# pasqualedem/LabelAnything

Hardware: AMD Instinct MI355X
Metric: episodes/sec (query+support fwd) ViT-B 1024px 1-shot (higher is better)
Workload: dtype f16; 1 GPU; BASELINE cfg2: SAM ViT-B 1024px encoder + LabelAnything decoder, 1-way 1-shot episodes (2 images each), random-init weights, full-resolution logits; parallelism=episode-sharded x1, no collective, launch=hipGraph replay

## Files before the change

labelanything_amd/csrc/attn_enc.hip:

```cpp
#include <cstdlib>
#include "la_common.h"
#ifndef LA_ATTN_ABL
#ifndef LA_ATTN_DMA_RUN
#define LA_ATTN_DMA_RUN 1
#endif
#define LA_ATTN_ABL 0
#endif
#ifndef LA_WIN_ROT
#define LA_WIN_ROT 1
#endif
#ifndef LA_WIN_HALF
#define LA_WIN_HALF 1
#endif
#ifndef LA_ATTN_X
#define LA_ATTN_X 0
#endif
#include "../../include/la_hip.h"
#include "attn_plan.h"

namespace la {

constexpr int HD = 64;
constexpr float NEG_BIG = -1.0e30f;
constexpr float RESCALE_THR = 8.0f;

template <typename T, int NH>
__global__ __launch_bounds__(256) void relpos_kernel(const T* __restrict__ qkv, int B, int heads, int G, int E,
                                                     const T* __restrict__ tabh, const T* __restrict__ tabw,
                                                     float* __restrict__ relh, float* __restrict__ relw) {
  const int w = blockIdx.x * 4 + (threadIdx.x >> 6);
  if (w >= B * heads * G) return;
  const int lane = threadIdx.x & 63, fr = lane & 31, fh = lane >> 5;
  const int y = w % G, bh = w / G, h = bh % heads, b = bh / heads;
  const int T_ = G * G;
  const int ntx = (G + 31) >> 5;
  const uint4 zero = make_uint4(0, 0, 0, 0);

  constexpr int HDT = 64 * NH, KS = 4 * NH;
  uint4 af[2][KS];
#pragma unroll
  for (int ti = 0; ti < 2; ++ti) {
    const int x = ti * 32 + fr;
    const bool ok = (ti < ntx) && (x < G);
    const T* p = qkv + ((size_t)b * T_ + (size_t)y * G + (ok ? x : 0)) * (3 * E) + h * HDT + fh * 8;
#pragma unroll
    for (int ks = 0; ks < KS; ++ks) af[ti][ks] = ok ? *reinterpret_cast<const uint4*>(p + ks * 16) : zero;
  }
  const size_t obase = ((size_t)bh * T_ + (size_t)y * G) * G;

  for (int tj = 0; tj < ntx; ++tj) {
    const int j = tj * 32 + fr;
    const bool okj = j < G;
    const T* p = tabh + (size_t)(okj ? (y - j + G - 1) : 0) * HDT + fh * 8;
    uint4 wf[KS];
#pragma unroll
    for (int ks = 0; ks < KS; ++ks) wf[ks] = okj ? *reinterpret_cast<const uint4*>(p + ks * 16) : zero;
#pragma unroll
    for (int ti = 0; ti < 2; ++ti) {
      if (ti >= ntx) continue;
      f32x16 acc;
#pragma unroll
      for (int r = 0; r < 16; ++r) acc[r] = 0.f;
#pragma unroll
      for (int ks = 0; ks < KS; ++ks) acc = Half16<T>::mfma32(af[ti][ks], wf[ks], acc);
#pragma unroll
      for (int r = 0; r < 16; ++r) {
        const int x = ti * 32 + (r & 3) + 8 * (r >> 2) + 4 * fh;
        if (x < G && okj) relh[obase + (size_t)x * G + j] = acc[r];
      }
    }
  }
  const int nrel = 2 * G - 1;
  const int ntr = (nrel + 31) >> 5;
  for (int tj = 0; tj < ntr; ++tj) {
    const int rp = tj * 32 + fr;
    const bool okr = rp < nrel;
    const T* p = tabw + (size_t)(okr ? rp : 0) * HDT + fh * 8;
    uint4 wf[KS];
#pragma unroll
    for (int ks = 0; ks < KS; ++ks) wf[ks] = okr ? *reinterpret_cast<const uint4*>(p + ks * 16) : zero;
#pragma unroll
    for (int ti = 0; ti < 2; ++ti) {
      if (ti >= ntx) continue;
      f32x16 acc;
#pragma unroll
      for (int r = 0; r < 16; ++r) acc[r] = 0.f;
#pragma unroll
      for (int ks = 0; ks < KS; ++ks) acc = Half16<T>::mfma32(af[ti][ks], wf[ks], acc);
#pragma unroll
      for (int r = 0; r < 16; ++r) {
        const int x = ti * 32 + (r & 3) + 8 * (r >> 2) + 4 * fh;
        const int kw = x + G - 1 - rp;
        if (x < G && okr && kw >= 0 && kw < G) relw[obase + (size_t)x * G + kw] = acc[r];
      }
    }
  }
}


__device__ __forceinline__ float xhalf_max(float v) {
  const auto r = __builtin_amdgcn_permlane32_swap(__float_as_uint(v), __float_as_uint(v), false, false);
  return fmaxf(__uint_as_float(r[0]), __uint_as_float(r[1]));
}
__device__ __forceinline__ float xhalf_sum(float v) {
  const auto r = __builtin_amdgcn_permlane32_swap(__float_as_uint(v), __float_as_uint(v), false, false);
  return __uint_as_float(r[0]) + __uint_as_float(r[1]);
}

#ifdef LA_DEBUG
__device__ unsigned long long g_win_stamps[4 * 16];
#define WIN_STAMP(i)                                                                                  \
  do {                                                                                                \
    if (MODE == ATTN_TABLES_WIN16 && blockIdx.x == gridDim.x / 2) {                                   \
      unsigned long long t_;                                                                          \
      asm volatile("s_memtime %0\n\ts_waitcnt lgkmcnt(0)" : "=s"(t_)::"memory");                     \
      if ((threadIdx.x & 63) == 0) g_win_stamps[(threadIdx.x >> 6) * 16 + (i)] = t_;                   \
    }                                                                                                 \
  } while (0)
#else
#define WIN_STAMP(i) do {} while (0)
#endif

struct AttnArgs {
  const void* qkv;
  const void* vt;
  void* out;
  const float* relh;
  const float* relw;
  const void* tabh;
  const void* tabw;
  int B, heads, T, Tpad, G, E;
  float scale;
  float* lse;
  float* cspart;
  int csH, csW;
  int imgH, imgW;
  const void* padrow;
  int nwx, nwin;
  unsigned mg_heads, mg_nwin, mg_nwx, mg_G;
};

__device__ __forceinline__ int udiv_magic(int n, int d, unsigned magic) { return d == 1 ? n : (int)__umulhi((unsigned)n, magic); }
static inline unsigned magic_of(int d) { return d <= 1 ? 0u : (unsigned)((0x100000000ull + (unsigned)d - 1) / (unsigned)d); }
static inline void set_win_magic(AttnArgs& a) {
  a.nwx = a.imgH > 0 ? (a.imgW + a.G - 1) / a.G : 1;
  a.nwin = a.imgH > 0 ? a.nwx * ((a.imgH + a.G - 1) / a.G) : 1;
  a.mg_heads = magic_of(a.heads);
  a.mg_nwin = magic_of(a.nwin);
  a.mg_nwx = magic_of(a.nwx);
  a.mg_G = magic_of(a.G);
}

template <typename T, int MODE, int NH, bool VROW = false>
__global__ __launch_bounds__(256, (((MODE == ATTN_TABLES_ROW64 || MODE == ATTN_TABLES_WIN16) && NH == 1) ? 3 : 2)) void attn_fwd_kernel(AttnArgs a) {
  constexpr bool WIN16 = MODE == ATTN_TABLES_WIN16;
  constexpr bool ROW64 = MODE == ATTN_TERMS_ROW64 || MODE == ATTN_TABLES_ROW64;
  constexpr int HDT = 64 * NH, KS = 4 * NH, SUB = 64 * 64 * 2, KVS = KV_STAGE * NH;
  extern __shared__ __attribute__((aligned(16))) char smem[];
  WIN_STAMP(0);
  const int tid = threadIdx.x, lane = tid & 63, wave = tid >> 6;
  const int fr = lane & 31, fh = lane >> 5;
  const int BH = a.B * a.heads;
  int bh, qblk;
  {
    const int nq = (a.T + 127) / 128;
    if (WIN16) {
      const bool two = nq == 2;
      if ((BH & 7) == 0) {
        const int idx = blockIdx.x >> 3;
        qblk = two ? (idx & 1) : 0;
        bh = ((two ? idx >> 1 : idx) << 3) + (blockIdx.x & 7);
      } else {
        qblk = (int)blockIdx.x >= BH;
        bh = blockIdx.x - (qblk ? BH : 0);
      }
    } else if ((BH & 7) == 0) {
      const int idx = blockIdx.x >> 3;
      qblk = idx % nq;
      bh = (idx / nq) * 8 + (blockIdx.x & 7);
    } else {
      bh = blockIdx.x % BH;
      qblk = blockIdx.x / BH;
    }
  }
  const int b = WIN16 ? udiv_magic(bh, a.heads, a.mg_heads) : bh / a.heads;
  const int h = bh - b * a.heads;
  const int T_ = a.T, E3 = 3 * a.E;
  const T* qkv = reinterpret_cast<const T*>(a.qkv);
  const T* vt = reinterpret_cast<const T*>(a.vt);
  const int q0 = qblk * 128 + ((WIN16 && LA_WIN_ROT) ? ((wave + bh) & 3) : wave) * 32;
  const int q = q0 + fr;
  const int qc = min(q, T_ - 1);
  const float inv_scale = 1.0f / a.scale;
  const float c2 = a.scale * 1.44269504088896340736f;
  const bool img_order = WIN16 && VROW && a.imgH > 0;
  int wimg = 0, wy0 = 0, wx0 = 0;
  if (img_order) {
    wimg = udiv_magic(b, a.nwin, a.mg_nwin);
    const int w_ = b - wimg * a.nwin;
    const int wy = udiv_magic(w_, a.nwx, a.mg_nwx);
    wy0 = wy * a.G;
    wx0 = (w_ - wy * a.nwx) * a.G;
  }
  const int qy5 = WIN16 ? udiv_magic(qc, a.G, a.mg_G) : 0, qx5 = qc - qy5 * a.G;
  auto img_row = [&](int ty, int tx) -> long {
    const int y = wy0 + ty, x = wx0 + tx;
    return (y < a.imgH && x < a.imgW) ? ((long)wimg * a.imgH + y) * a.imgW + x : -1;
  };
  long qrow = (long)b * T_ + qc;
  if (img_order) qrow = img_row(qy5, qx5);
  const T* padrow = reinterpret_cast<const T*>(a.padrow);
  if (img_order && a.lse == nullptr && wy0 + udiv_magic(qblk * 128, a.G, a.mg_G) >= a.imgH) {
    if (a.cspart != nullptr && tid < HDT) a.cspart[((size_t)b * ((T_ + 127) / 128) + qblk) * a.E + h * HDT + tid] = 0.f;
    return;
  }

  uint4 qf[KS];
  {
    const T* p = (qrow >= 0 ? qkv + (size_t)qrow * E3 : padrow) + h * HDT + fh * 8;
#pragma unroll
    for (int ks = 0; ks < KS; ++ks) qf[ks] = *reinterpret_cast<const uint4*>(p + ks * 16);
  }

  const T* ksrc[2];
  const T* vsrc[2];
  int krow[2], koff[2], voff[2];
#pragma unroll
  for (int i = 0; i < 2; ++i) {
    const int row = (i * 4 + wave) * 8 + (lane >> 3);
    const int chunk = (lane & 7) ^ ((row >> 1) & 7);
    krow[i] = row;
    koff[i] = a.E + h * HDT + chunk * 8;
    voff[i] = 2 * a.E + h * HDT + ((lane & 7) ^ (4 * ((row >> 1) & 1))) * 8;
    ksrc[i] = qkv + (size_t)b * T_ * E3 + koff[i];
    vsrc[i] = VROW ? qkv + (size_t)b * T_ * E3 + voff[i] : vt + ((size_t)bh * HDT + row) * a.Tpad + chunk * 8;
  }
  const unsigned lds0 = lds_addr_of(smem);
  const T* img_base = qkv + (size_t)b * T_ * E3;
  unsigned krun[2], vrun[2];
#pragma unroll
  for (int i = 0; i < 2; ++i) {
    krun[i] = (unsigned)(((size_t)krow[i] * E3 + koff[i]) * sizeof(T));
    vrun[i] = (unsigned)(((size_t)krow[i] * E3 + voff[i]) * sizeof(T));
  }
  const unsigned tile_step = (unsigned)((size_t)64 * E3 * sizeof(T));
  auto dma = [&](int j, int stage) {
    const unsigned sk = lds0 + stage * KVS;
    const unsigned sv = sk + NH * SUB;
#pragma unroll
    for (int i = 0; i < 2; ++i) {
      int key = 0;
      const T* kp = nullptr;
      const T* vp = nullptr;
      if (!WIN16 && !LA_ATTN_DMA_RUN) {
        key = min(j * 64 + krow[i], T_ - 1);
        kp = ksrc[i] + (size_t)key * E3;
        if (VROW) vp = vsrc[i] + (size_t)key * E3;
      } else if (!WIN16) {
        unsigned ko = krun[i], vo = vrun[i];
        if (j * 64 + 64 > T_) {
          const unsigned back = (unsigned)max(j * 64 + krow[i] - (T_ - 1), 0) * (unsigned)(E3 * sizeof(T));
          ko -= back;
          vo -= back;
        }
        krun[i] += tile_step;
        vrun[i] += tile_step;
#pragma unroll
        for (int hh = 0; hh < NH; ++hh) {
          dma16s(img_base, ko + hh * 128, sk + hh * SUB + (i * 4 + wave) * 1024);
          if (VROW) dma16s(img_base, vo + hh * 128, sv + hh * SUB + (i * 4 + wave) * 1024);
          else dma16(vsrc[i] + (size_t)hh * 64 * a.Tpad + j * 64, sv + hh * SUB + (i * 4 + wave) * 1024);
        }
        continue;
      } else if (WIN16) {
        const int slot = j * 64 + krow[i];
        const int ty = min(slot >> 4, a.G - 1), tx = min(slot & 15, a.G - 1);
        key = ty * a.G + tx;
        if (img_order) {
          const long r = img_row(ty, tx);
          const T* rp = r >= 0 ? qkv + (size_t)r * E3 : padrow;
          kp = rp + koff[i];
          vp = rp + voff[i];
        }
      }
      if (WIN16 && !img_order) {
        kp = ksrc[i] + (size_t)key * E3;
        if (VROW) vp = vsrc[i] + (size_t)key * E3;
      }
#pragma unroll
      for (int hh = 0; hh < NH; ++hh) {
        dma16(kp + hh * 64, sk + hh * SUB + (i * 4 + wave) * 1024);
        if (VROW) dma16(vp + hh * 64, sv + hh * SUB + (i * 4 + wave) * 1024);
        else dma16(vsrc[i] + (size_t)hh * 64 * a.Tpad + j * 64, sv + hh * SUB + (i * 4 + wave) * 1024);
      }
    }
  };

  const int ntiles = WIN16 ?((16 * a.G + 63) >> 6) : ((T_ + 63) >> 6);
  const bool half_last = WIN16 && LA_WIN_HALF && ((16 * a.G) & 63) != 0 && ((16 * a.G) & 63) <= 32;
  dma(0, 0);
  WIN_STAMP(1);

  float* bias_lds = reinterpret_cast<float*>(smem + 2 * KVS);
  f32x16 rw[2];
  float bw8[8];
  float* my_bh = nullptr;
  float* my_bw = nullptr;
  const int* keyinfo = nullptr;
  if (MODE == ATTN_TERMS_ROW64) {
    my_bh = bias_lds + wave * 32 * 65;
    for (int i = 0; i < 32; ++i) {
      const int qi = min(q0 + i, T_ - 1);
      my_bh[i * 65 + lane] = a.relh[((size_t)bh * T_ + qi) * 64 + lane] * inv_scale;
    }
    const float* p = a.relw + ((size_t)bh * T_ + qc) * 64;
#pragma unroll
    for (int t = 0; t < 2; ++t)
#pragma unroll
      for (int g4 = 0; g4 < 4; ++g4) {
        const float4 v = *reinterpret_cast<const float4*>(p + t * 32 + 8 * g4 + 4 * fh);
        rw[t][g4 * 4 + 0] = v.x * inv_scale;
        rw[t][g4 * 4 + 1] = v.y * inv_scale;
        rw[t][g4 * 4 + 2] = v.z * inv_scale;
        rw[t][g4 * 4 + 3] = v.w * inv_scale;
      }
  } else if (WIN16) {
    const int G = a.G, nrel = 2 * G - 1;
    my_bh = bias_lds + wave * 32 * 33;
    const T* th = reinterpret_cast<const T*>(a.tabh) + (size_t)min(fr, nrel - 1) * HDT + fh * 8;
    const T* tw = reinterpret_cast<const T*>(a.tabw) + (size_t)min(fr, nrel - 1) * HDT + fh * 8;
    f32x16 uh, uw;
#pragma unroll
    for (int r = 0; r < 16; ++r) uh[r] = uw[r] = 0.f;
#pragma unroll
    for (int ks = 0; ks < KS; ++ks) {
      uh = Half16<T>::mfma32(*reinterpret_cast<const uint4*>(th + ks * 16), qf[ks], uh);
      uw = Half16<T>::mfma32(*reinterpret_cast<const uint4*>(tw + ks * 16), qf[ks], uw);
    }
#pragma unroll
    for (int r = 0; r < 16; ++r) my_bh[fr * 33 + (r & 3) + 8 * (r >> 2) + 4 * fh] = uw[r] * inv_scale;
    __builtin_amdgcn_wave_barrier();
    const int qx = qx5;
#pragma unroll
    for (int i = 0; i < 8; ++i) {
      const int kw = 8 * (i >> 2) + 4 * fh + (i & 3);
      bw8[i] = (kw < G) ? my_bh[fr * 33 + qx + G - 1 - kw] : NEG_BIG;
    }
    __builtin_amdgcn_wave_barrier();
#pragma unroll
    for (int r = 0; r < 16; ++r) my_bh[fr * 33 + (r & 3) + 8 * (r >> 2) + 4 * fh] = uh[r] * inv_scale;
    __builtin_amdgcn_wave_barrier();
  } else if (MODE == ATTN_TABLES_ROW64) {
    my_bh = bias_lds + wave * 32 * 33;
    const int x0 = q0 & 63;
    const T* tabw = reinterpret_cast<const T*>(a.tabw);
#pragma unroll
    for (int t = 0; t < 2; ++t)
#pragma unroll
      for (int r = 0; r < 16; ++r) rw[t][r] = 0.f;
#pragma unroll 1
    for (int tt = 0; tt < 3; ++tt) {
      const T* tp = tabw + (size_t)min(x0 + tt * 32 + fr, 126) * HDT + fh * 8;
      f32x16 u;
#pragma unroll
      for (int r = 0; r < 16; ++r) u[r] = 0.f;
#pragma unroll
      for (int ks = 0; ks < KS; ++ks) u = Half16<T>::mfma32(*reinterpret_cast<const uint4*>(tp + ks * 16), qf[ks], u);
      __builtin_amdgcn_wave_barrier();
#pragma unroll
      for (int r = 0; r < 16; ++r) my_bh[fr * 33 + (r & 3) + 8 * (r >> 2) + 4 * fh] = u[r] * inv_scale;
      __builtin_amdgcn_wave_barrier();
#pragma unroll
      for (int t = 0; t < 2; ++t)
#pragma unroll
        for (int r = 0; r < 16; ++r) {
          const int kw = t * 32 + (r & 3) + 8 * (r >> 2) + 4 * fh;
          const int i = fr + 63 - kw - tt * 32;
          if (i >= 0 && i < 32) rw[t][r] = my_bh[fr * 33 + i];
        }
    }
    __builtin_amdgcn_wave_barrier();
  } else if (MODE == ATTN_TERMS) {
    const int G = a.G, GS = G + 1;
    my_bh = bias_lds + wave * 2 * 32 * GS;
    my_bw = my_bh + 32 * GS;
    for (int idx = lane; idx < 32 * G; idx += 64) {
      const int i = idx / G, k = idx % G;
      const size_t src = ((size_t)bh * T_ + min(q0 + i, T_ - 1)) * G + k;
      my_bh[i * GS + k] = a.relh[src] * inv_scale;
      my_bw[i * GS + k] = a.relw[src] * inv_scale;
    }
    int* ki = reinterpret_cast<int*>(bias_lds + 4 * 2 * 32 * GS);
    for (int k = tid; k < a.Tpad; k += 256) ki[k] = ((k / G) << 16) | (k % G);
    keyinfo = ki;
  } else if (MODE == ATTN_TABLES_WIN) {
    const int G = a.G, nrel = 2 * G - 1;
    my_bh = bias_lds + wave * 2 * 32 * 33;
    my_bw = my_bh + 32 * 33;
    const T* th = reinterpret_cast<const T*>(a.tabh) + (size_t)min(fr, nrel - 1) * HDT + fh * 8;
    const T* tw = reinterpret_cast<const T*>(a.tabw) + (size_t)min(fr, nrel - 1) * HDT + fh * 8;
    f32x16 uh, uw;
#pragma unroll
    for (int r = 0; r < 16; ++r) uh[r] = uw[r] = 0.f;
#pragma unroll
    for (int ks = 0; ks < KS; ++ks) {
      uh = Half16<T>::mfma32(*reinterpret_cast<const uint4*>(th + ks * 16), qf[ks], uh);
      uw = Half16<T>::mfma32(*reinterpret_cast<const uint4*>(tw + ks * 16), qf[ks], uw);
    }
#pragma unroll
    for (int r = 0; r < 16; ++r) {
      const int row = (r & 3) + 8 * (r >> 2) + 4 * fh;
      my_bh[fr * 33 + row] = uh[r] * inv_scale;
      my_bw[fr * 33 + row] = uw[r] * inv_scale;
    }
    int* ki = reinterpret_cast<int*>(bias_lds + 4 * 2 * 32 * 33);
    for (int k = tid; k < a.Tpad; k += 256) {
      const int kk = min(k, T_ - 1);
      ki[k] = ((G - 1 - kk / G) << 16) | (G - 1 - kk % G);
    }
    keyinfo = ki;
  }

  f32x16 oacc[2 * NH];
#pragma unroll
  for (int d = 0; d < 2 * NH; ++d)
#pragma unroll
    for (int r = 0; r < 16; ++r) oacc[d][r] = 0.f;
  float m_run = NEG_BIG, l_run = 0.f;
  unsigned vtr[2] = {0u, 0u};
  if (VROW) {
    const int j = (lane & 15) >> 2, c = lane & 3, jb = (j >> 1) & 1, gd = (lane >> 4) & 1;
#pragma unroll
    for (int dd = 0; dd < 2; ++dd) vtr[dd] = (unsigned)((8 * fh + j) * 128 + ((4 * (dd ^ jb) + 2 * gd + (c >> 1)) << 4) + (c & 1) * 8);
  }

  WIN_STAMP(2);
  dma_wait<0>();
  auto fill_relh_half = [&](int hf) {
    const int y = q0 >> 6;
    const T* tp = reinterpret_cast<const T*>(a.tabh) + (size_t)min(y + (1 - hf) * 32 + fr, 126) * HDT + fh * 8;
    f32x16 u;
#pragma unroll
    for (int r = 0; r < 16; ++r) u[r] = 0.f;
#pragma unroll
    for (int ks = 0; ks < KS; ++ks) u = Half16<T>::mfma32(*reinterpret_cast<const uint4*>(tp + ks * 16), qf[ks], u);
    __builtin_amdgcn_wave_barrier();
#pragma unroll
    for (int r = 0; r < 16; ++r) my_bh[fr * 33 + 31 - ((r & 3) + 8 * (r >> 2) + 4 * fh)] = u[r] * inv_scale;
    __builtin_amdgcn_wave_barrier();
  };
  if (MODE == ATTN_TABLES_ROW64) fill_relh_half(0);
  __syncthreads();
  WIN_STAMP(3);
  const bool idle_wave = q0 >= T_;
  for (int j = 0; j < ntiles; ++j) {
#if !(LA_ATTN_ABL & 8)
    if (j + 1 < ntiles) dma(j + 1, (j + 1) & 1);
#endif
    if (idle_wave) {
      dma_wait<0>();
      __syncthreads();
      continue;
    }
    const char* sk = smem + (j & 1) * KVS;
    const char* sv = sk + NH * SUB;
    if (MODE == ATTN_TABLES_ROW64 && j == 32) fill_relh_half(1);

    f32x16 s[2];
    float rh = 0.f;
    const bool half = WIN16 && half_last && j == ntiles - 1;
    if (MODE == ATTN_TERMS_ROW64) rh = my_bh[fr * 65 + j];
    if (MODE == ATTN_TABLES_ROW64) rh = my_bh[fr * 33 + (j & 31)];
#pragma unroll
    for (int t = 0; t < 2; ++t) {
      if (WIN16 && t == 1 && half) continue;
      const uint4 kf0 = *reinterpret_cast<const uint4*>(sk + swz_off(t * 32 + fr, fh));
      if (ROW64) {
        s[t] = Half16<T>::mfma32(kf0, qf[0], rw[t]);
      } else if (WIN16) {
        f32x16 z;
        const int qy = qy5;
#pragma unroll
        for (int hh = 0; hh < 2; ++hh) {
          const int kh = 4 * j + 2 * t + hh;
          const float bh = (kh < a.G) ? my_bh[fr * 33 + qy + a.G - 1 - kh] : NEG_BIG;
#pragma unroll
          for (int i = 0; i < 8; ++i) z[hh * 8 + i] = bh + bw8[i];
        }
        s[t] = Half16<T>::mfma32(kf0, qf[0], z);
      } else {
        f32x16 z;
#pragma unroll
        for (int r = 0; r < 16; ++r) z[r] = 0.f;
        s[t] = Half16<T>::mfma32(kf0, qf[0], z);
      }
    }
#if !(LA_ATTN_ABL & 2)
#pragma unroll
    for (int ks = 1; ks < KS; ++ks) {
#pragma unroll
      for (int t = 0; t < 2; ++t) {
        if (WIN16 && t == 1 && half) continue;
        const uint4 kf = *reinterpret_cast<const uint4*>(sk + (ks >> 2) * SUB + swz_off(t * 32 + fr, (ks & 3) * 2 + fh));
        s[t] = Half16<T>::mfma32(kf, qf[ks], s[t]);
      }
    }
#endif
    if (MODE == ATTN_TERMS) {
      const int GS = a.G + 1;
#pragma unroll
      for (int t = 0; t < 2; ++t)
#pragma unroll
        for (int r = 0; r < 16; ++r) {
          const int key = j * 64 + t * 32 + (r & 3) + 8 * (r >> 2) + 4 * fh;
          const int info = keyinfo[key];
          s[t][r] += my_bh[fr * GS + (info >> 16)] + my_bw[fr * GS + (info & 0xffff)];
        }
    }
    if (MODE == ATTN_TABLES_WIN) {
      const int qy = qc / a.G, qx = qc % a.G;
      const float* bh_q = my_bh + fr * 33 + qy;
      const float* bw_q = my_bw + fr * 33 + qx;
#pragma unroll
      for (int t = 0; t < 2; ++t)
#pragma unroll
        for (int r = 0; r < 16; ++r) {
          const int key = j * 64 + t * 32 + (r & 3) + 8 * (r >> 2) + 4 * fh;
          const int info = keyinfo[key];
          s[t][r] += bh_q[info >> 16] + bw_q[info & 0xffff];
        }
    }
    if (!WIN16 && j * 64 + 64 > T_) {
#pragma unroll
      for (int t = 0; t < 2; ++t)
#pragma unroll
        for (int r = 0; r < 16; ++r) {
          const int key = j * 64 + t * 32 + (r & 3) + 8 * (r >> 2) + 4 * fh;
          if (key >= T_) s[t][r] = NEG_BIG;
        }
    }

#if LA_ATTN_X & 2
    if (j == 0) {
#endif
    float mx = s[0][0];
#pragma unroll
    for (int t = 0; t < 2; ++t) {
      if (WIN16 && t == 1 && half) continue;
#pragma unroll
      for (int r = 0; r < 16; ++r) mx = fmaxf(mx, s[t][r]);
    }
    mx = xhalf_max(mx) + rh;
    if (!__all((mx - m_run) * c2 <= RESCALE_THR)) {
      const float m_new = fmaxf(m_run, mx);
      const float alpha = __builtin_amdgcn_exp2f((m_run - m_new) * c2);
      l_run *= alpha;
#pragma unroll
      for (int d = 0; d < 2 * NH; ++d)
#pragma unroll
        for (int r = 0; r < 16; ++r) oacc[d][r] *= alpha;
      m_run = m_new;
    }
#if LA_ATTN_X & 2
    }
#endif
    const float mc = (rh - m_run) * c2;
    float psum = 0.f;
#pragma unroll
    for (int t = 0; t < 2; ++t) {
      if (WIN16 && t == 1 && half) continue;
#pragma unroll
      for (int r = 0; r < 16; ++r) {
#if LA_ATTN_ABL & 1
        const float p = fmaf(s[t][r], c2, mc);
#else
#if LA_ATTN_X & 4
        const float p = __builtin_amdgcn_exp2f(s[t][r]);
#else
        const float p = __builtin_amdgcn_exp2f(fmaf(s[t][r], c2, mc));
#endif
#endif
        s[t][r] = p;
#if !(LA_ATTN_X & 8)
        psum += p;
#endif
      }
    }
    l_run += psum;

    uint4 pf[4];
#pragma unroll
    for (int ks = 0; ks < 4; ++ks) {
      if (WIN16 && ks >= 2 && half) continue;
      const int t = ks >> 1, g0 = (ks & 1) * 8;
      const uint32_t x0 = pack2<T>(s[t][g0 + 0], s[t][g0 + 1]);
      const uint32_t x1 = pack2<T>(s[t][g0 + 2], s[t][g0 + 3]);
      const uint32_t y0 = pack2<T>(s[t][g0 + 4], s[t][g0 + 5]);
      const uint32_t y1 = pack2<T>(s[t][g0 + 6], s[t][g0 + 7]);
      const auto r0 = __builtin_amdgcn_permlane32_swap(x0, y0, false, false);
      const auto r1 = __builtin_amdgcn_permlane32_swap(x1, y1, false, false);
      pf[ks] = make_uint4(r0[0], r1[0], r0[1], r1[1]);
    }

#if LA_ATTN_ABL & 4
    asm volatile("" ::"v"(pf[0].x), "v"(pf[0].y), "v"(pf[0].z), "v"(pf[0].w), "v"(pf[1].x), "v"(pf[1].y), "v"(pf[1].z), "v"(pf[1].w));
    asm volatile("" ::"v"(pf[2].x), "v"(pf[2].y), "v"(pf[2].z), "v"(pf[2].w), "v"(pf[3].x), "v"(pf[3].y), "v"(pf[3].z), "v"(pf[3].w));
#else
#pragma unroll
    for (int ks = 0; ks < 4; ++ks) {
      if (WIN16 && ks >= 2 && half) continue;
#pragma unroll
      for (int d = 0; d < 2 * NH; ++d) {
        uint4 vf;
        if (VROW) {
          typedef short s16x4 __attribute__((ext_vector_type(4)));
          typedef __attribute__((address_space(3))) s16x4* lds_s16x4;
          const unsigned va = lds_addr_of(sv) + (d >> 1) * SUB + vtr[d & 1] + ks * 2048;
          const s16x4 lo = __builtin_amdgcn_ds_read_tr16_b64_v4i16((lds_s16x4)(uintptr_t)va);
          const s16x4 hi = __builtin_amdgcn_ds_read_tr16_b64_v4i16((lds_s16x4)(uintptr_t)(va + 512));
          const uint2 l2 = __builtin_bit_cast(uint2, lo), h2 = __builtin_bit_cast(uint2, hi);
          vf = make_uint4(l2.x, l2.y, h2.x, h2.y);
        } else {
          vf = *reinterpret_cast<const uint4*>(sv + (d >> 1) * SUB + swz_off((d & 1) * 32 + fr, ks * 2 + fh));
        }
        oacc[d] = Half16<T>::mfma32(vf, pf[ks], oacc[d]);
      }
    }
#endif

#if !(LA_ATTN_ABL & 8)
    if (j < 4) WIN_STAMP(8 + j);
    dma_wait<0>();
    __syncthreads();
#endif
    if (j < 4) WIN_STAMP(4 + j);
  }

  const float l_tot = xhalf_sum(l_run);
  const float inv_l = 1.0f / l_tot;
  if (a.lse != nullptr && q < T_ && fh == 0) a.lse[(size_t)bh * a.Tpad + q] = m_run * c2 + __builtin_amdgcn_logf(l_tot);
  if (q < T_ && qrow >= 0) {
    T* op = reinterpret_cast<T*>(a.out) + (size_t)qrow * a.E + h * HDT;
#pragma unroll
    for (int d = 0; d < 2 * NH; ++d)
#pragma unroll
      for (int g4 = 0; g4 < 4; ++g4) {
        uint2 v;
        v.x = pack2<T>(oacc[d][g4 * 4 + 0] * inv_l, oacc[d][g4 * 4 + 1] * inv_l);
        v.y = pack2<T>(oacc[d][g4 * 4 + 2] * inv_l, oacc[d][g4 * 4 + 3] * inv_l);
        *reinterpret_cast<uint2*>(op + d * 32 + 8 * g4 + 4 * fh) = v;
      }
  }
  WIN_STAMP(12);
  if (a.cspart != nullptr) {
    bool valid = q < T_ && qrow >= 0;
    if (WIN16 && a.csH > 0 && !img_order) {
      const int nwx = (a.csW + a.G - 1) / a.G, nwy = (a.csH + a.G - 1) / a.G;
      const int w = b % (nwx * nwy);
      valid = valid && (w / nwx) * a.G + qy5 < a.csH && (w % nwx) * a.G + qx5 < a.csW;
    }
    char* tile = smem + wave * (NH * 4096);
#pragma unroll
    for (int d = 0; d < 2 * NH; ++d)
#pragma unroll
      for (int g4 = 0; g4 < 4; ++g4) {
        uint2 v;
        v.x = pack2<T>(oacc[d][g4 * 4 + 0] * inv_l, oacc[d][g4 * 4 + 1] * inv_l);
        v.y = pack2<T>(oacc[d][g4 * 4 + 2] * inv_l, oacc[d][g4 * 4 + 3] * inv_l);
        if (!valid) v = make_uint2(0u, 0u);
        const int c16 = 4 * (d & 1) + g4;
        *reinterpret_cast<uint2*>(tile + (d >> 1) * 4096 + fr * 128 + ((c16 ^ (4 * ((fr >> 1) & 1))) << 4) + 8 * fh) = v;
      }
    asm volatile("s_waitcnt lgkmcnt(0)" ::: "memory");
    __builtin_amdgcn_wave_barrier();
    unsigned ctr[2];
    {
      const int j = (lane & 15) >> 2, c = lane & 3, jb = (j >> 1) & 1, gd = (lane >> 4) & 1;
#pragma unroll
      for (int dd = 0; dd < 2; ++dd) ctr[dd] = (unsigned)((8 * fh + j) * 128 + ((4 * (dd ^ jb) + 2 * gd + (c >> 1)) << 4) + (c & 1) * 8);
    }
    const uint32_t one2 = pack2<T>(1.0f, 1.0f);
    const uint4 ones = make_uint4(one2, one2, one2, one2);
    float* red = reinterpret_cast<float*>(smem + 4 * NH * 4096);
#pragma unroll
    for (int d = 0; d < 2 * NH; ++d) {
      f32x16 cs;
#pragma unroll
      for (int r = 0; r < 16; ++r) cs[r] = 0.f;
#pragma unroll
      for (int ks = 0; ks < 2; ++ks) {
        typedef short s16x4 __attribute__((ext_vector_type(4)));
        typedef __attribute__((address_space(3))) s16x4* lds_s16x4;
        const unsigned va = lds_addr_of(tile) + (d >> 1) * 4096 + ctr[d & 1] + ks * 2048;
        const s16x4 lo = __builtin_amdgcn_ds_read_tr16_b64_v4i16((lds_s16x4)(uintptr_t)va);
        const s16x4 hi = __builtin_amdgcn_ds_read_tr16_b64_v4i16((lds_s16x4)(uintptr_t)(va + 512));
        const uint2 l2 = __builtin_bit_cast(uint2, lo), h2 = __builtin_bit_cast(uint2, hi);
        cs = Half16<T>::mfma32(make_uint4(l2.x, l2.y, h2.x, h2.y), ones, cs);
      }
      if (fr == 0) {
#pragma unroll
        for (int r = 0; r < 16; ++r) red[wave * HDT + d * 32 + (r & 3) + 8 * (r >> 2) + 4 * fh] = cs[r];
      }
    }
    __syncthreads();
    if (tid < HDT) {
      float t = 0.f;
#pragma unroll
      for (int w = 0; w < 4; ++w) t += red[w * HDT + tid];
      const int nq = (T_ + 127) / 128;
      a.cspart[((size_t)b * nq + qblk) * a.E + h * HDT + tid] = t;
    }
  }
}


template <typename T>
__global__ __launch_bounds__(256, 3) void attn_window_kernel(AttnArgs a, int qtiles) {
  extern __shared__ __attribute__((aligned(16))) char smem[];
  const int tid = threadIdx.x, lane = tid & 63, wave = tid >> 6;
  const int fr = lane & 31, fh = lane >> 5;
  const int G = a.G, T_ = a.T, E3 = 3 * a.E;
  int* keyinfo = reinterpret_cast<int*>(smem);
  for (int k = tid; k < a.Tpad; k += 256) {
    const int kk = min(k, T_ - 1);
    keyinfo[k] = ((G - 1 - kk / G) << 16) | (G - 1 - kk % G);
  }
  __syncthreads();
  const int job = blockIdx.x * 4 + wave;
  const int njobs = a.B * a.heads * qtiles;
  if (job >= njobs) return;
  const int qt = job % qtiles, bh = job / qtiles;
  const int h = bh % a.heads, b = bh / a.heads;
  const T* qkv = reinterpret_cast<const T*>(a.qkv);
  const T* vt = reinterpret_cast<const T*>(a.vt);
  const int q0 = qt * 32, q = q0 + fr, qc = min(q, T_ - 1);
  const float inv_scale = 1.0f / a.scale;
  const float c2 = a.scale * 1.44269504088896340736f;

  uint4 qf[4];
  {
    const T* p = qkv + ((size_t)b * T_ + qc) * E3 + h * HD + fh * 8;
#pragma unroll
    for (int ks = 0; ks < 4; ++ks) qf[ks] = *reinterpret_cast<const uint4*>(p + ks * 16);
  }
  float* my_bh = reinterpret_cast<float*>(smem + a.Tpad * sizeof(int)) + wave * 2 * 32 * 33;
  float* my_bw = my_bh + 32 * 33;
  {
    const int nrel = 2 * G - 1;
    const T* th = reinterpret_cast<const T*>(a.tabh) + (size_t)min(fr, nrel - 1) * HD + fh * 8;
    const T* tw = reinterpret_cast<const T*>(a.tabw) + (size_t)min(fr, nrel - 1) * HD + fh * 8;
    f32x16 uh, uw;
#pragma unroll
    for (int r = 0; r < 16; ++r) uh[r] = uw[r] = 0.f;
#pragma unroll
    for (int ks = 0; ks < 4; ++ks) {
      uh = Half16<T>::mfma32(*reinterpret_cast<const uint4*>(th + ks * 16), qf[ks], uh);
      uw = Half16<T>::mfma32(*reinterpret_cast<const uint4*>(tw + ks * 16), qf[ks], uw);
    }
#pragma unroll
    for (int r = 0; r < 16; ++r) {
      const int row = (r & 3) + 8 * (r >> 2) + 4 * fh;
      my_bh[fr * 33 + row] = uh[r] * inv_scale;
      my_bw[fr * 33 + row] = uw[r] * inv_scale;
    }
    __builtin_amdgcn_wave_barrier();
  }
  const float* bh_q = my_bh + fr * 33 + qc / G;
  const float* bw_q = my_bw + fr * 33 + qc % G;

  const T* kbase = qkv + (size_t)b * T_ * E3 + a.E + h * HD + fh * 8;
  const T* vbase = vt + ((size_t)bh * HD + fr) * a.Tpad + fh * 8;
  f32x16 oacc[2];
#pragma unroll
  for (int d = 0; d < 2; ++d)
#pragma unroll
    for (int r = 0; r < 16; ++r) oacc[d][r] = 0.f;
  float m_run = NEG_BIG, l_run = 0.f;
  const int ntiles = (T_ + 63) >> 6;
  for (int j = 0; j < ntiles; ++j) {
    f32x16 s[2];
#pragma unroll
    for (int t = 0; t < 2; ++t) {
      const T* kp = kbase + (size_t)min(j * 64 + t * 32 + fr, T_ - 1) * E3;
      uint4 kf[4];
#pragma unroll
      for (int ks = 0; ks < 4; ++ks) kf[ks] = *reinterpret_cast<const uint4*>(kp + ks * 16);
#pragma unroll
      for (int r = 0; r < 16; ++r) s[t][r] = 0.f;
#pragma unroll
      for (int ks = 0; ks < 4; ++ks) s[t] = Half16<T>::mfma32(kf[ks], qf[ks], s[t]);
    }
    uint4 vf[2][4];
#pragma unroll
    for (int d = 0; d < 2; ++d)
#pragma unroll
      for (int ks = 0; ks < 4; ++ks) vf[d][ks] = *reinterpret_cast<const uint4*>(vbase + (size_t)d * 32 * a.Tpad + j * 64 + ks * 16);
#pragma unroll
    for (int t = 0; t < 2; ++t)
#pragma unroll
      for (int r = 0; r < 16; ++r) {
        const int key = j * 64 + t * 32 + (r & 3) + 8 * (r >> 2) + 4 * fh;
        const int info = keyinfo[key];
        const float sv = s[t][r] + bh_q[info >> 16] + bw_q[info & 0xffff];
        s[t][r] = (key < T_) ? sv : NEG_BIG;
      }
    float mx = s[0][0];
// ... 145 lines not shown
          if (key >= T_) s[t][r] = NEG_BIG;
        }
    }
    float mx = s[0][0];
#pragma unroll
    for (int t = 0; t < 2; ++t)
#pragma unroll
      for (int r = 0; r < 16; ++r) mx = fmaxf(mx, s[t][r]);
    mx = xhalf_max(mx);
    if (!__all((mx - m_run) * c2 <= RESCALE_THR)) {
      const float m_new = fmaxf(m_run, mx);
      const float alpha = __builtin_amdgcn_exp2f((m_run - m_new) * c2);
      l_run *= alpha;
#pragma unroll
      for (int d = 0; d < 2; ++d)
#pragma unroll
        for (int r = 0; r < 16; ++r) oacc[d][r] *= alpha;
      m_run = m_new;
    }
    const float mc = -m_run * c2;
    float psum = 0.f;
#pragma unroll
    for (int t = 0; t < 2; ++t)
#pragma unroll
      for (int r = 0; r < 16; ++r) {
        const float p = __builtin_amdgcn_exp2f(fmaf(s[t][r], c2, mc));
        s[t][r] = p;
        psum += p;
      }
    l_run += psum;
    uint4 pf[4];
#pragma unroll
    for (int ks = 0; ks < 4; ++ks) {
      const int t = ks >> 1, g0 = (ks & 1) * 8;
      const uint32_t x0 = pack2<T>(s[t][g0 + 0], s[t][g0 + 1]);
      const uint32_t x1 = pack2<T>(s[t][g0 + 2], s[t][g0 + 3]);
      const uint32_t y0 = pack2<T>(s[t][g0 + 4], s[t][g0 + 5]);
      const uint32_t y1 = pack2<T>(s[t][g0 + 6], s[t][g0 + 7]);
      const auto r0 = __builtin_amdgcn_permlane32_swap(x0, y0, false, false);
      const auto r1 = __builtin_amdgcn_permlane32_swap(x1, y1, false, false);
      pf[ks] = make_uint4(r0[0], r1[0], r0[1], r1[1]);
    }
#pragma unroll
    for (int ks = 0; ks < 4; ++ks)
#pragma unroll
      for (int d = 0; d < 2; ++d) {
        const uint4 vf = *reinterpret_cast<const uint4*>(sv + swz_off(d * 32 + fr, ks * 2 + fh));
        oacc[d] = Half16<T>::mfma32(vf, pf[ks], oacc[d]);
      }
    dma_wait<0>();
    __syncthreads();
  }
  const float l_tot = xhalf_sum(l_run);
  const float inv_l = 1.0f / l_tot;
  if (q < T_) {
    T* op = reinterpret_cast<T*>(a.out) + ((size_t)b * T_ + q) * a.E + h * 64;
#pragma unroll
    for (int d = 0; d < 2; ++d)
#pragma unroll
      for (int g4 = 0; g4 < 4; ++g4) {
        uint2 v;
        v.x = pack2<T>(oacc[d][g4 * 4 + 0] * inv_l, oacc[d][g4 * 4 + 1] * inv_l);
        v.y = pack2<T>(oacc[d][g4 * 4 + 2] * inv_l, oacc[d][g4 * 4 + 3] * inv_l);
        *reinterpret_cast<uint2*>(op + d * 32 + 8 * g4 + 4 * fh) = v;
      }
  }
}

template <typename T>
__global__ __launch_bounds__(256) void qk_fp8_kernel(const T* __restrict__ qkv, long rows, int E, unsigned char* __restrict__ out) {
  const int per_row = (2 * E) / 8;
  for (long i = (long)blockIdx.x * 256 + threadIdx.x; i < rows * per_row; i += (long)gridDim.x * 256) {
    const long r = i / per_row;
    const int c = (int)(i % per_row) * 8;
    const uint4 v = *reinterpret_cast<const uint4*>(qkv + r * 3 * E + c);
    const T* e = reinterpret_cast<const T*>(&v);
    unsigned w0 = 0, w1 = 0;
    w0 = __builtin_amdgcn_cvt_pk_fp8_f32((float)e[0], (float)e[1], w0, false);
    w0 = __builtin_amdgcn_cvt_pk_fp8_f32((float)e[2], (float)e[3], w0, true);
    w1 = __builtin_amdgcn_cvt_pk_fp8_f32((float)e[4], (float)e[5], w1, false);
    w1 = __builtin_amdgcn_cvt_pk_fp8_f32((float)e[6], (float)e[7], w1, true);
    *reinterpret_cast<uint2*>(out + r * 2 * E + c) = make_uint2(w0, w1);
  }
}

static int attn_fwd_plan_checked(int entry, const LaAttnCall& c, LaAttnPlan* p) {
  char err[384];
  if (attn_fwd_plan(entry, c, p, err, sizeof(err)) != 0) {
    la_set_error("%s", err);
    return -1;
  }
#ifdef LA_DEBUG
  static const char* wforce = getenv("LA_WINDOW_PATH");
  if (wforce && wforce[0] == 'l' && p->launch[0].kernel == LA_ATTN_K_WINDOW) p->launch[0] = attn_fwd_tile_launch(ATTN_TABLES_WIN, false, c);
#endif
  return 0;
}

static LaAttnCall attn_call(int B, int heads, int T, int Tpad, int G, int E, int mode, int dt) {
  LaAttnCall c{};
  c.B = B, c.heads = heads, c.T = T, c.Tpad = Tpad, c.G = G, c.E = E, c.mode = mode, c.dt = dt;
  return c;
}

static int attn_fwd_run(int entry, const LaAttnCall& c, float scale, void* stream) {
  LaAttnPlan p;
  if (attn_fwd_plan_checked(entry, c, &p) != 0) return -1;
  AttnArgs a{c.qkv, c.vt, const_cast<void*>(c.out16), (const float*)c.relh, (const float*)c.relw, c.tabh, c.tabw, c.B, c.heads, c.T, c.Tpad, c.G,
             c.E, scale, (float*)c.lse, (float*)c.cspart, c.csH, c.csW};
  if (p.launch[0].mode == ATTN_TABLES_WIN16) {
    if (c.imgH > 0) a.imgH = c.imgH, a.imgW = c.imgW, a.padrow = c.padrow;
    set_win_magic(a);
  }
  hipStream_t st = reinterpret_cast<hipStream_t>(stream);
  if (c.dt == LA_F16) launch_attn_fwd<f16_t>(p, a, st);
  else launch_attn_fwd<bf16_t>(p, a, st);
  LA_CHECK_LAUNCH(attn_entry_name(entry));
  return 0;
}

}

extern "C" int la_attn_fwd_plan(int entry, const LaAttnCall* call, LaAttnPlan* out) {
  LA_CHECK_ARG(call && out, "la_attn_fwd_plan: null pointer");
  return la::attn_fwd_plan_checked(entry, *call, out);
}

extern "C" int la_relpos_terms(const void* qkv, int B, int heads, int G, int E, const void* tabh, const void* tabw, float* relh,
                               float* relw, int dt, void* stream) {
  LA_CHECK_ARG(qkv && tabh && tabw && relh && relw, "la_relpos_terms: null pointer");
  LA_CHECK_ARG(B > 0 && heads > 0 && G > 0 && G <= 64 && (E == heads * 64 || E == heads * 128),
               "la_relpos_terms: needs head_dim 64 or 128 and G <= 64 (G=%d E=%d heads=%d)", G, E, heads);
  LA_CHECK_ARG(dt == LA_F16 || dt == LA_BF16, "la_relpos_terms: bad dtype %d", dt);
  const int waves = B * heads * G;
  hipStream_t st = reinterpret_cast<hipStream_t>(stream);
  const dim3 grid((waves + 3) / 4), blk(256);
  const bool wide = E == heads * 128;
  if (dt == LA_F16) {
    if (wide) hipLaunchKernelGGL((la::relpos_kernel<la::f16_t, 2>), grid, blk, 0, st, (const la::f16_t*)qkv, B, heads, G, E, (const la::f16_t*)tabh, (const la::f16_t*)tabw, relh, relw);
    else hipLaunchKernelGGL((la::relpos_kernel<la::f16_t, 1>), grid, blk, 0, st, (const la::f16_t*)qkv, B, heads, G, E, (const la::f16_t*)tabh, (const la::f16_t*)tabw, relh, relw);
  } else {
    if (wide) hipLaunchKernelGGL((la::relpos_kernel<la::bf16_t, 2>), grid, blk, 0, st, (const la::bf16_t*)qkv, B, heads, G, E, (const la::bf16_t*)tabh, (const la::bf16_t*)tabw, relh, relw);
    else hipLaunchKernelGGL((la::relpos_kernel<la::bf16_t, 1>), grid, blk, 0, st, (const la::bf16_t*)qkv, B, heads, G, E, (const la::bf16_t*)tabh, (const la::bf16_t*)tabw, relh, relw);
  }
  LA_CHECK_LAUNCH("la_relpos_terms");
  return 0;
}

#ifdef LA_DEBUG
extern "C" int la_dbg_win_stamps(unsigned long long* host_out) {
  (void)hipDeviceSynchronize();
  return (int)hipMemcpyFromSymbol(host_out, HIP_SYMBOL(la::g_win_stamps), sizeof(unsigned long long) * 64);
}
#endif

extern "C" int la_attn_fwd_cs(const void* qkv, const void* vt, void* out16, const float* relh, const float* relw, const void* tabh,
                              const void* tabw, int B, int heads, int T, int Tpad, int G, int E, float scale, int mode, float* cspart, int csH,
                              int csW, int dt, void* stream) {
  LaAttnCall c = la::attn_call(B, heads, T, Tpad, G, E, mode, dt);
  c.qkv = qkv, c.vt = vt, c.out16 = out16, c.relh = relh, c.relw = relw, c.tabh = tabh, c.tabw = tabw;
  c.cspart = cspart, c.csH = csH, c.csW = csW;
  return la::attn_fwd_run(LA_ATTN_EP_FWD, c, scale, stream);
}

extern "C" int la_attn_fwd(const void* qkv, const void* vt, void* out16, const float* relh, const float* relw, const void* tabh,
                           const void* tabw, int B, int heads, int T, int Tpad, int G, int E, float scale, int mode, int dt, void* stream) {
  return la_attn_fwd_cs(qkv, vt, out16, relh, relw, tabh, tabw, B, heads, T, Tpad, G, E, scale, mode, nullptr, 0, 0, dt, stream);
}

extern "C" int la_attn_fwd_rows(const void* qkv, void* out16, const void* tabh, const void* tabw, int B, int heads, int T, int Tpad, int G, int E,
                                float scale, int mode, float* cspart, int imgH, int imgW, const void* padrow, int dt, void* stream) {
  LaAttnCall c = la::attn_call(B, heads, T, Tpad, G, E, mode, dt);
  c.qkv = qkv, c.out16 = out16, c.tabh = tabh, c.tabw = tabw, c.cspart = cspart;
  c.imgH = imgH, c.imgW = imgW, c.padrow = padrow;
  return la::attn_fwd_run(LA_ATTN_EP_FWD_ROWS, c, scale, stream);
}

extern "C" int la_attn_fwd_lse(const void* qkv, const void* vt, void* out16, float* lse, int B, int heads, int T, int Tpad, int E, float scale,
                               int dt, void* stream) {
  LaAttnCall c = la::attn_call(B, heads, T, Tpad, 0, E, LA_ATTN_PLAIN, dt);
  c.qkv = qkv, c.vt = vt, c.out16 = out16, c.lse = lse;
  return la::attn_fwd_run(LA_ATTN_EP_FWD_LSE, c, scale, stream);
}

extern "C" int la_attn_fwd_relpos_lse(const void* qkv, const void* vt, void* out16, const float* relh, const float* relw, float* lse, int B, int heads,
                                      int T, int Tpad, int G, int E, float scale, int dt, void* stream) {
  LaAttnCall c = la::attn_call(B, heads, T, Tpad, G, E, LA_ATTN_RELPOS, dt);
  c.qkv = qkv, c.vt = vt, c.out16 = out16, c.relh = relh, c.relw = relw, c.lse = lse;
  return la::attn_fwd_run(LA_ATTN_EP_FWD_RELPOS_LSE, c, scale, stream);
}

extern "C" int la_qk_fp8(const void* qkv, long rows, int E, void* qk8, int dt, void* stream) {
  LA_CHECK_ARG(qkv && qk8 && rows > 0 && E > 0 && (E % 8) == 0 && (dt == LA_F16 || dt == LA_BF16), "la_qk_fp8: bad arguments");
  hipStream_t st = reinterpret_cast<hipStream_t>(stream);
  const long n = rows * (2 * E / 8);
  const dim3 grid((unsigned)((n + 255) / 256 > 8192 ? 8192 : (n + 255) / 256)), blk(256);
  if (dt == LA_F16) hipLaunchKernelGGL(la::qk_fp8_kernel<la::f16_t>, grid, blk, 0, st, (const la::f16_t*)qkv, rows, E, (unsigned char*)qk8);
  else hipLaunchKernelGGL(la::qk_fp8_kernel<la::bf16_t>, grid, blk, 0, st, (const la::bf16_t*)qkv, rows, E, (unsigned char*)qk8);
  LA_CHECK_LAUNCH("la_qk_fp8");
  return 0;
}

extern "C" int la_attn_fwd_fp8(const void* qk8, const void* vt, void* out16, int B, int heads, int T, int Tpad, int E, float scale, int dt,
                               void* stream) {
  LA_CHECK_ARG(qk8 && vt && out16, "la_attn_fwd_fp8: null pointer");
  LA_CHECK_ARG(B > 0 && heads > 0 && T > 0 && E == heads * 64, "la_attn_fwd_fp8: needs head_dim 64 (E=%d heads=%d)", E, heads);
  LA_CHECK_ARG(Tpad >= T && (Tpad % 64) == 0, "la_attn_fwd_fp8: Tpad=%d must be a multiple of 64 covering T=%d", Tpad, T);
  LA_CHECK_ARG(dt == LA_F16 || dt == LA_BF16, "la_attn_fwd_fp8: bad dtype %d", dt);
  la::AttnArgs a{nullptr, vt, out16, nullptr, nullptr, nullptr, nullptr, B, heads, T, Tpad, 0, E, scale, nullptr};
  hipStream_t st = reinterpret_cast<hipStream_t>(stream);
  const int nblk = (T + 127) / 128 * B * heads;
  constexpr int LDS = 2 * (64 * 64 + 64 * 64 * 2);
  if (dt == LA_F16) hipLaunchKernelGGL(la::attn_fwd_fp8_kernel<la::f16_t>, dim3(nblk), dim3(256), LDS, st, a, (const unsigned char*)qk8);
  else hipLaunchKernelGGL(la::attn_fwd_fp8_kernel<la::bf16_t>, dim3(nblk), dim3(256), LDS, st, a, (const unsigned char*)qk8);
  LA_CHECK_LAUNCH("la_attn_fwd_fp8");
  return 0;
}
```

Before: 392.6 episodes/s.

## Interleave next-tile K/V DMA issue into softmax loop for non-window attention

Splits the DMA into an address-computation step and a piecewise issue step. For non-window modes (the default is STAGE_AT=1), the four K/V copy pieces of the next tile are now issued one at a time between softmax row groups instead of all at the top of the tile. The aim is to hide DMA issue cost behind the exp math. The last tile is peeled into its own compile-time specialization, and the wave index is made scalar via readfirstlane. Debug-only per-tile timestamps are also added. In exchange, the scheduling barriers can restrict how the compiler interleaves instructions.

```diff
diff --git a/labelanything_amd/csrc/attn_enc.hip b/labelanything_amd/csrc/attn_enc.hip
--- a/labelanything_amd/csrc/attn_enc.hip
+++ b/labelanything_amd/csrc/attn_enc.hip
@@ -11,6 +11,9 @@
 #endif
 #ifndef LA_WIN_HALF
 #define LA_WIN_HALF 1
+#endif
+#ifndef LA_ATTN_STAGE_AT
+#define LA_ATTN_STAGE_AT 1
 #endif
 #ifndef LA_ATTN_X
 #define LA_ATTN_X 0
@@ -114,11 +117,22 @@
     if (MODE == ATTN_TABLES_WIN16 && blockIdx.x == gridDim.x / 2) {                                   \
       unsigned long long t_;                                                                          \
       asm volatile("s_memtime %0\n\ts_waitcnt lgkmcnt(0)" : "=s"(t_)::"memory");                     \
-      if ((threadIdx.x & 63) == 0) g_win_stamps[(threadIdx.x >> 6) * 16 + (i)] = t_;                   \
+      win_log = (int)(threadIdx.x & 63) == (i) ? t_ : win_log;                                        \
     }                                                                                                 \
+  } while (0)
+__device__ unsigned g_tile_stamps[2 * 4 * 64];
+#define TILE_STAMP(p)                                                                                                         \
+  do {                                                                                                                        \
+    if ((MODE == ATTN_TABLES_WIN16 || MODE == ATTN_TABLES_ROW64) && blockIdx.x == gridDim.x / 2 &&                            \
+        (unsigned)(j - tile_j0) < 8u) {                                                                                       \
+      unsigned long long t_;                                                                                                  \
+      asm volatile("s_memtime %0\n\ts_waitcnt lgkmcnt(0)" : "=s"(t_)::"memory");                                             \
+      tile_log = lane == (j - tile_j0) * 8 + (p) ? (unsigned)t_ : tile_log;                                                  \
+    }                                                                                                                         \
   } while (0)
 #else
 #define WIN_STAMP(i) do {} while (0)
+#define TILE_STAMP(p) do {} while (0)
 #endif
 
 struct AttnArgs {
@@ -157,8 +171,12 @@
   constexpr bool ROW64 = MODE == ATTN_TERMS_ROW64 || MODE == ATTN_TABLES_ROW64;
   constexpr int HDT = 64 * NH, KS = 4 * NH, SUB = 64 * 64 * 2, KVS = KV_STAGE * NH;
   extern __shared__ __attribute__((aligned(16))) char smem[];
+#ifdef LA_DEBUG
+  unsigned long long win_log = 0ull;
+#endif
   WIN_STAMP(0);
-  const int tid = threadIdx.x, lane = tid & 63, wave = tid >> 6;
+  const int tid = threadIdx.x, lane = tid & 63;
+  const int wave = __builtin_amdgcn_readfirstlane(tid >> 6);
   const int fr = lane & 31, fh = lane >> 5;
   const int BH = a.B * a.heads;
   int bh, qblk;
@@ -244,60 +262,66 @@
     vrun[i] = (unsigned)(((size_t)krow[i] * E3 + voff[i]) * sizeof(T));
   }
   const unsigned tile_step = (unsigned)((size_t)64 * E3 * sizeof(T));
-  auto dma = [&](int j, int stage) {
-    const unsigned sk = lds0 + stage * KVS;
-    const unsigned sv = sk + NH * SUB;
+  const T* src_k[2] = {nullptr, nullptr};
+  const T* src_v[2] = {nullptr, nullptr};
+  auto dma_src = [&](int j) {
 #pragma unroll
     for (int i = 0; i < 2; ++i) {
       int key = 0;
-      const T* kp = nullptr;
-      const T* vp = nullptr;
       if (!WIN16 && !LA_ATTN_DMA_RUN) {
         key = min(j * 64 + krow[i], T_ - 1);
-        kp = ksrc[i] + (size_t)key * E3;
-        if (VROW) vp = vsrc[i] + (size_t)key * E3;
+        src_k[i] = ksrc[i] + (size_t)key * E3;
+        if (VROW) src_v[i] = vsrc[i] + (size_t)key * E3;
       } else if (!WIN16) {
-        unsigned ko = krun[i], vo = vrun[i];
         if (j * 64 + 64 > T_) {
           const unsigned back = (unsigned)max(j * 64 + krow[i] - (T_ - 1), 0) * (unsigned)(E3 * sizeof(T));
-          ko -= back;
-          vo -= back;
+          krun[i] -= back;
+          vrun[i] -= back;
         }
-        krun[i] += tile_step;
-        vrun[i] += tile_step;
-#pragma unroll
-        for (int hh = 0; hh < NH; ++hh) {
-          dma16s(img_base, ko + hh * 128, sk + hh * SUB + (i * 4 + wave) * 1024);
-          if (VROW) dma16s(img_base, vo + hh * 128, sv + hh * SUB + (i * 4 + wave) * 1024);
-          else dma16(vsrc[i] + (size_t)hh * 64 * a.Tpad + j * 64, sv + hh * SUB + (i * 4 + wave) * 1024);
-        }
-        continue;
-      } else if (WIN16) {
+      } else {
         const int slot = j * 64 + krow[i];
         const int ty = min(slot >> 4, a.G - 1), tx = min(slot & 15, a.G - 1);
         key = ty * a.G + tx;
         if (img_order) {
           const long r = img_row(ty, tx);
           const T* rp = r >= 0 ? qkv + (size_t)r * E3 : padrow;
-          kp = rp + koff[i];
-          vp = rp + voff[i];
+          src_k[i] = rp + koff[i];
+          src_v[i] = rp + voff[i];
+        } else {
+          src_k[i] = ksrc[i] + (size_t)key * E3;
+          if (VROW) src_v[i] = vsrc[i] + (size_t)key * E3;
         }
       }
-      if (WIN16 && !img_order) {
-        kp = ksrc[i] + (size_t)key * E3;
-        if (VROW) vp = vsrc[i] + (size_t)key * E3;
-      }
+    }
+  };
+  auto dma = [&](int j, int stage, int pieces = 15) {
+    const unsigned sk = lds0 + stage * KVS;
+    const unsigned sv = sk + NH * SUB;
+    constexpr bool RUN = !WIN16 && LA_ATTN_DMA_RUN;
+#pragma unroll
+    for (int i = 0; i < 2; ++i) {
+      const bool do_k = (pieces >> i) & 1, do_v = (pieces >> (2 + i)) & 1;
+      const unsigned dst = (i * 4 + wave) * 1024;
 #pragma unroll
       for (int hh = 0; hh < NH; ++hh) {
-        dma16(kp + hh * 64, sk + hh * SUB + (i * 4 + wave) * 1024);
-        if (VROW) dma16(vp + hh * 64, sv + hh * SUB + (i * 4 + wave) * 1024);
-        else dma16(vsrc[i] + (size_t)hh * 64 * a.Tpad + j * 64, sv + hh * SUB + (i * 4 + wave) * 1024);
-      }
+        if (do_k) {
+          if (RUN) dma16s(img_base, krun[i] + hh * 128, sk + hh * SUB + dst);
+          else dma16(src_k[i] + hh * 64, sk + hh * SUB + dst);
+        }
+        if (do_v) {
+          if (!VROW) dma16(vsrc[i] + (size_t)hh * 64 * a.Tpad + j * 64, sv + hh * SUB + dst);
+          else if (RUN) dma16s(img_base, vrun[i] + hh * 128, sv + hh * SUB + dst);
+          else dma16(src_v[i] + hh * 64, sv + hh * SUB + dst);
+        }
+      }
+      if (RUN && do_k) krun[i] += tile_step;
+      if (RUN && do_v) vrun[i] += tile_step;
     }
   };
 
   const int ntiles = WIN16 ?((16 * a.G + 63) >> 6) : ((T_ + 63) >> 6);
   const bool half_last = WIN16 && LA_WIN_HALF && ((16 * a.G) & 63) != 0 && ((16 * a.G) & 63) <= 32;
+  dma_src(0);
   dma(0, 0);
   WIN_STAMP(1);
 
@@ -453,14 +477,29 @@
   __syncthreads();
   WIN_STAMP(3);
   const bool idle_wave = q0 >= T_;
-  for (int j = 0; j < ntiles; ++j) {
-#if !(LA_ATTN_ABL & 8)
-    if (j + 1 < ntiles) dma(j + 1, (j + 1) & 1);
-#endif
+#ifdef LA_DEBUG
+  unsigned tile_log = 0u;
+  const int tile_j0 = WIN16 ? 0 : 28;
+#endif
+  auto tile = [&](const int j, auto last_tile) {
+    constexpr bool LAST = decltype(last_tile)::value;
+    TILE_STAMP(0);
+    constexpr bool stage_next = !LAST && !(LA_ATTN_ABL & 8);
+    constexpr bool stage_in_softmax = LA_ATTN_STAGE_AT == 2 || (LA_ATTN_STAGE_AT == 1 && !WIN16);
+    if (stage_next) dma_src(j + 1);
+    if (stage_next && (!stage_in_softmax || idle_wave)) dma(j + 1, (j + 1) & 1);
+    auto stage_piece = [&](int p) {
+      if (stage_in_softmax && stage_next) {
+        __builtin_amdgcn_sched_barrier(0);
+        dma(j + 1, (j + 1) & 1, 1 << p);
+        __builtin_amdgcn_sched_barrier(0);
+      }
+    };
+    if (!stage_in_softmax) TILE_STAMP(1);
     if (idle_wave) {
       dma_wait<0>();
       __syncthreads();
-      continue;
+      return;
     }
     const char* sk = smem + (j & 1) * KVS;
     const char* sv = sk + NH * SUB;
@@ -468,7 +507,7 @@
 
     f32x16 s[2];
     float rh = 0.f;
-    const bool half = WIN16 && half_last && j == ntiles - 1;
+    const bool half = WIN16 && LAST && half_last;
     if (MODE == ATTN_TERMS_ROW64) rh = my_bh[fr * 65 + j];
     if (MODE == ATTN_TABLES_ROW64) rh = my_bh[fr * 33 + (j & 31)];
 #pragma unroll
@@ -506,6 +545,7 @@
       }
     }
 #endif
+    TILE_STAMP(2);
     if (MODE == ATTN_TERMS) {
       const int GS = a.G + 1;
 #pragma unroll
@@ -567,10 +607,13 @@
     const float mc = (rh - m_run) * c2;
     float psum = 0.f;
 #pragma unroll
-    for (int t = 0; t < 2; ++t) {
+    for (int tg = 0; tg < 4; ++tg) {
+      stage_piece(tg);
+      if (stage_in_softmax && tg == 3) TILE_STAMP(1);
+      const int t = tg >> 1;
       if (WIN16 && t == 1 && half) continue;
 #pragma unroll
-      for (int r = 0; r < 16; ++r) {
+      for (int r = (tg & 1) * 8; r < (tg & 1) * 8 + 8; ++r) {
 #if LA_ATTN_ABL & 1
         const float p = fmaf(s[t][r], c2, mc);
 #else
@@ -601,6 +644,7 @@
       const auto r1 = __builtin_amdgcn_permlane32_swap(x1, y1, false, false);
       pf[ks] = make_uint4(r0[0], r1[0], r0[1], r1[1]);
     }
+    TILE_STAMP(3);
 
 #if LA_ATTN_ABL & 4
     asm volatile("" ::"v"(pf[0].x), "v"(pf[0].y), "v"(pf[0].z), "v"(pf[0].w), "v"(pf[1].x), "v"(pf[1].y), "v"(pf[1].z), "v"(pf[1].w));
@@ -627,14 +671,23 @@
       }
     }
 #endif
+    TILE_STAMP(4);
 
 #if !(LA_ATTN_ABL & 8)
     if (j < 4) WIN_STAMP(8 + j);
     dma_wait<0>();
+    TILE_STAMP(5);
     __syncthreads();
 #endif
+    TILE_STAMP(6);
     if (j < 4) WIN_STAMP(4 + j);
-  }
+  };
+  for (int j = 0; j + 1 < ntiles; ++j) tile(j, std::false_type{});
+  tile(ntiles - 1, std::true_type{});
+#ifdef LA_DEBUG
+  if ((MODE == ATTN_TABLES_WIN16 || MODE == ATTN_TABLES_ROW64) && blockIdx.x == gridDim.x / 2)
+    g_tile_stamps[((MODE == ATTN_TABLES_WIN16 ? 1 : 0) * 4 + wave) * 64 + lane] = tile_log;
+#endif
 
   const float l_tot = xhalf_sum(l_run);
   const float inv_l = 1.0f / l_tot;
@@ -652,6 +705,9 @@
       }
   }
   WIN_STAMP(12);
+#ifdef LA_DEBUG
+  if (MODE == ATTN_TABLES_WIN16 && blockIdx.x == gridDim.x / 2 && lane < 16) g_win_stamps[wave * 16 + lane] = win_log;
+#endif
   if (a.cspart != nullptr) {
     bool valid = q < T_ && qrow >= 0;
     if (WIN16 && a.csH > 0 && !img_order) {
@@ -1103,6 +1159,10 @@
   (void)hipDeviceSynchronize();
   return (int)hipMemcpyFromSymbol(host_out, HIP_SYMBOL(la::g_win_stamps), sizeof(unsigned long long) * 64);
 }
+extern "C" int la_dbg_tile_stamps(unsigned* host_out) {
+  (void)hipDeviceSynchronize();
+  return (int)hipMemcpyFromSymbol(host_out, HIP_SYMBOL(la::g_tile_stamps), sizeof(unsigned) * 512);
+}
 #endif
 
 extern "C" int la_attn_fwd_cs(const void* qkv, const void* vt, void* out16, const float* relh, const float* relw, const void* tabh,
```

Result: faster. 396.5 episodes/s (median of 6 runs) (+1.0%).
